# uber/aresdb

Hardware: NVIDIA H100
Metric: rows/s, 1e9-row time-bucketed SUM group-by (cfg3) (higher is better)
Workload: dtype u32/u16/u8 filters; f32 fares summed into f64 (exactly, as integers on the 2^-S grid the zone map allows)

## Files before the change

### aresdb_b200/csrc/batch_plan.cu

```cuda
#include <cooperative_groups.h>
#include <algorithm>
#include <memory>
#include <vector>

#include "agg.cuh"
#include "column.cuh"
#include "dimrow.cuh"
#include "fused_device.cuh"
#include "plan_device.cuh"
#include "radix_sort.cuh"
#include "scan.cuh"
#include "small_sort.cuh"

namespace cg = cooperative_groups;

namespace aresb {

ForeignDesc makeForeignDesc(const ForeignColumnVector &f);
void gatherDims(const uint8_t *in, const DimLayout &Lin, const uint32_t *rows, int g, uint8_t *out,
                const DimLayout &Lout, cudaStream_t s);
int hllRegisterVectors(const uint64_t *hash, const uint32_t *values, uint32_t *index, int R, uint8_t **hllVectorPtr,
                       size_t *hllVectorSizePtr, uint16_t **hllDimRegIDCountPtr, cudaStream_t s);
int reduceByHash(const uint64_t *hash, const uint32_t *index, const uint8_t *measures, int width, AggOp op, int n,
                 uint32_t *outIndex, uint8_t *outValues, cudaStream_t s, uint64_t *outHash = nullptr);
// ... 2021 lines not shown
CGoCallResHandle AggStateFinalizeHLL(void *state, uint8_t **dimValuesPtr, uint8_t **hllVectorPtr, size_t *hllVectorSizePtr,
                                     uint16_t **hllDimRegIDCountPtr, void *cudaStream, int device) {
  return guarded("AggStateFinalizeHLL", device, [&]() -> int64_t {
    return finalizeHLL(asState(state), dimValuesPtr, hllVectorPtr, hllVectorSizePtr, hllDimRegIDCountPtr,
                       (cudaStream_t)cudaStream);
  });
}

CGoCallResHandle AggStateReset(void *state, void *cudaStream, int device) {
  return guarded("AggStateReset", device, [&]() -> int64_t {
    AggState *st = asState(state);
    cudaStream_t s = (cudaStream_t)cudaStream;
    resetClaimedKernel<<<smCount() * 4, 256, 0, s>>>(st->table, st->accNeutral);
    checkLastError("AggStateReset");
    ARES_CUDA(cudaMemsetAsync(st->table.counters, 0, 256, s));
    st->occUpper = 0;
    st->unchecked = 0;
    st->everChecked = false;
    st->resultHost[8] = 0;
    return 0;
  });
}

CGoCallResHandle AresJitDryRun(AggSpec spec, const BatchPlan *plan, char **sourceOut) {
  CGoCallResHandle h = {nullptr, nullptr};
  try {
    AggState st;
    memset(&st.table, 0, sizeof(st.table));
    describeState(&st, spec);
    st.capacity = st.hllDense ? kHllDenseSlots : 0;
    static thread_local DevPlan P;
    compilePlan(&st, *plan, P);
    prepareInputs(P, *plan, nullptr, nullptr);
    layoutStages(P, spec.ExpectedGroups);
    std::string src;
    size_t n = jitCompileOnly(P, &src);
    if (sourceOut) *sourceOut = strdup(src.c_str());
    h.res = reinterpret_cast<void *>(n);
  } catch (const std::exception &e) {
    h.pStrErr = strdup((std::string("AresJitDryRun: ") + e.what()).c_str());
  }
  return h;
}

CGoCallResHandle AresJitDryRunMulti(const AggSpec *specs, int numSpecs, const BatchPlan *plan, char **sourceOut) {
  CGoCallResHandle h = {nullptr, nullptr};
  try {
    if (!specs || !plan || numSpecs < 1 || numSpecs > kJitMaxMeasures) throw EngineError("numSpecs must be 1.." + std::to_string(kJitMaxMeasures));
    std::vector<AggState> st(numSpecs);
    AggState *sts[kJitMaxMeasures];
    for (int k = 0; k < numSpecs; k++) {
      memset(&st[k].table, 0, sizeof(st[k].table));
      describeState(&st[k], specs[k]);
      st[k].capacity = 0;
      sts[k] = &st[k];
    }
    checkSharedStates(sts, numSpecs);
    static thread_local DevPlan P;
    MeasurePlans subs;
    if (numSpecs == 1) {
      compilePlan(sts[0], *plan, P);
      prepareInputs(P, *plan, nullptr, nullptr);
      layoutStages(P, specs[0].ExpectedGroups);
    } else if (!planShared(sts, numSpecs, *plan, P, subs, nullptr, nullptr)) {
      throw EngineError("this plan and zone map run one kernel per state (no shared direct-indexed form)");
    }
// ... 23 lines not shown
```

### aresdb_b200/csrc/jit.cu

```cuda
#include <dlfcn.h>

#include <cassert>
#include <mutex>
#include <sstream>
#include <unordered_map>
#include <vector>
#include <unistd.h>

#include "plan_device.cuh"
#include "jit_embedded.h"

namespace aresb {

typedef struct _nvrtcProgram *nvrtcProgram;
struct Nvrtc {
  int (*CreateProgram)(nvrtcProgram *, const char *, const char *, int, const char *const *, const char *const *);
  int (*CompileProgram)(nvrtcProgram, int, const char *const *);
  int (*GetProgramLogSize)(nvrtcProgram, size_t *);
  int (*GetProgramLog)(nvrtcProgram, char *);
  int (*GetCUBINSize)(nvrtcProgram, size_t *);
  int (*GetCUBIN)(nvrtcProgram, char *);
  int (*DestroyProgram)(nvrtcProgram *);
  bool ok = false;
};
// ... 163 lines not shown
          }
          if (filtered && I.sink == PLAN_SINK_MEASURE && !I.wide && I.nops == 1 && I.fn == Noop && I.akind == 1  && I.aclass == VC_F32 &&
              I.rclass == VC_F32 && I.oclass == VC_F64 && P.cols[I.acol].in.mode != 0 && P.cols[I.acol].rangeKnown) {
            const int e = (int)((P.cols[I.acol].rangeHi >> 23) & 0xFF);
            int S = e == 0 ? 60 : 31 - (e - 127);
            if (S > 60) S = 60;
            if (S < 0) continue;
            P.denseFx = 1;
            P.fxMeasureInst = (int8_t)i;
            P.fxShift = (int8_t)S;
          }
        }
      }
    }
  }
}

static int denseAccOf(uint8_t measWidth, uint8_t aggOp) { return measWidth == 4 && aggOp != OP_MIN_F32 && aggOp != OP_MAX_F32 ? 1 : 2; }
static bool positiveLiteralSum(const DevInst &I, uint8_t aggOp) {
  return I.sink == PLAN_SINK_MEASURE && !I.wide && (aggOp == OP_SUM_I32 || aggOp == OP_SUM_I64) && I.nops == 1 && I.fn == Noop &&
         I.akind == 2  && I.avalid && (I.aclass == VC_I32 || I.aclass == VC_U32) && (int32_t)I.aconst > 0;
}

static void generate(const DevPlan &P, const DevTable &G, Generated &out) {
  const int nmeas = P.nmeas > 1 ? P.nmeas : 1;
  const bool multi = nmeas > 1;
  assert(P.baseCounts == nullptr || P.tileBcBytes != 0 || P.skipCount);
  std::ostringstream os;
  JitParams &jp = out.params;
  memset(&jp, 0, sizeof(jp));
  jp.measureIdentity = P.measureIdentity;
  jp.accNeutral = P.accNeutral;
  jp.G = G;
  jp.ctaAcc = P.ctaAcc;
  jp.numFullTiles = P.numFullTiles;
  jp.numRows = P.numRows;
  jp.join = P.join;
  jp.resume = P.resume;
  jp.startCount = P.startCount;
  int nrle = 0;
  std::vector<int> rleSlot(P.ncols, -1);
  for (int c = 0; c < P.ncols; c++) {
    const DevColumn &col = P.cols[c];
    if (!col.rle) continue;
    assert(nrle < kJitMaxRle && (P.baseCounts == nullptr || P.tileBcBytes != 0));
    rleSlot[c] = nrle;
    jp.rle[nrle].counts = reinterpret_cast<const uint32_t *>(col.in.base);
    jp.rle[nrle].nulls = col.in.base + col.in.nullsOff;
    jp.rle[nrle].values = col.in.base + col.in.valuesOff;
    jp.rle[nrle].tileRun = col.tileRun;
    jp.rle[nrle].length = col.in.length;
    jp.rle[nrle].startBit = col.in.startBit;
    nrle++;
  }

  struct Part { uint32_t off, bytes, stride, isBits, startBit; };
  std::vector<Part> parts;
  size_t tx = 0;
  for (int c = 0; c < P.ncols; c++) {
    const DevColumn &col = P.cols[c];
    if (col.staged) {
      jp.partSrc[parts.size()] = col.in.base + col.in.valuesOff;
      parts.push_back({col.smemValues, col.tileValueBytes, col.width ? P.tileRows * col.width : P.tileRows / 8,
                       col.width ? 0u : 1u, col.in.startBit});
      tx += col.tileValueBytes;
    }
    if (col.hasNulls) {
      jp.partSrc[parts.size()] = col.in.base + col.in.nullsOff;
      parts.push_back({col.smemNulls, col.tileNullBytes, P.tileRows / 8, 1u, col.in.startBit});
      tx += col.tileNullBytes;
    }
  }
  if (P.tileBcBytes != 0) {
    jp.partSrc[parts.size()] = reinterpret_cast<const uint8_t *>(P.baseCounts);
    parts.push_back({P.smemBc, P.tileBcBytes, P.tileRows * 4u, 2u, 0u});
    tx += P.tileBcBytes;
  }
  const bool runLengths = P.tileBcBytes != 0 && !P.skipCount;
  const int kw = P.keyMode == 1  ? 4 : 1;

  struct DenseDim { int inst; bool viaQuot; bool nullCanon; uint32_t lo, cnt, step; bool span32; };
  std::vector<DenseDim> dense;
  std::vector<int> denseOfInst(P.ninsts, -1);
  const bool denseOkPlan = P.denseNd != 0;
  const bool denseOk = denseOkPlan;
  if (denseOk) {
    uint32_t stride = 1;
    for (int k = 0; k < P.denseNd; k++) {
      dense.push_back({P.denseInst[k], P.denseViaQuot[k] != 0, P.denseNullCanon[k] != 0, P.denseLo[k], P.denseCnt[k], P.denseStep[k],
                       P.denseSpan32[k] != 0});
      jp.dBase[k] = P.denseBase[k]; jp.dSpan[k] = P.denseSpan[k];
      jp.dMagic32[k] = P.denseSpan32[k] ? (uint32_t)((1ull << 32) / P.denseStep[k] + 1ull) : 0u;
      denseOfInst[P.denseInst[k]] = k;
      jp.dLo[k] = P.denseLo[k]; jp.dCnt[k] = P.denseCnt[k]; jp.dStep[k] = P.denseStep[k]; jp.dStride[k] = stride;
      stride *= P.denseCnt[k] + 1;
    }
    jp.dTotal = P.denseTotal;
    jp.gAcc = P.denseAcc;
    const uint32_t copyStride = (P.denseTotal + 15) / 16 * 16 + 1;
    uint32_t reps = 1;
    while (!P.denseGlobal && reps < 32 && (uint64_t)copyStride * reps * 2 <= P.smemSlots) reps *= 2;
    jp.dReps = reps;
    jp.dRepStride = reps > 1 ? copyStride : P.denseTotal;
    if (P.hll) { jp.dReps = 1; jp.dRepStride = P.denseTotal; }
    if (P.denseGlobal) {
      jp.dReps = P.denseGlobalReps ? P.denseGlobalReps : 1;
      jp.dRepStride = P.denseTotal;
    }
  }
  int denseAcc = denseAccOf(P.measWidth, P.aggOp);
  int fxMeasure = -1;
  if (denseOk && !P.denseGlobal && P.denseFx) {
    denseAcc = 4;
    fxMeasure = P.fxMeasureInst;
    jp.fxScale = ldexpf(1.0f, P.fxShift);
    jp.fxInv = ldexp(1.0, -P.fxShift);
  }
  bool denseFlags = true, denseCheck = P.neutralSafe;
  for (int i = 0; i < P.ninsts && !multi; i++) {
    if (positiveLiteralSum(P.insts[i], P.aggOp)) {
      denseCheck = false;
      denseFlags = false;
    }
  }
  if (fxMeasure >= 0) denseFlags = false;
  struct MeasForm { int inst, acc; bool flags, check, fx, runLengths; uint8_t aggOp; };
  std::vector<MeasForm> mf;
  if (multi) {
    for (int m = 0; m < nmeas; m++) {
      const DevMeasure &M = P.meas[m];
      const bool lit = positiveLiteralSum(P.insts[M.inst], M.aggOp);
      mf.push_back({M.inst, M.denseFx ? 4 : denseAccOf(M.measWidth, M.aggOp), !lit && !M.denseFx, M.neutralSafe && !lit, M.denseFx != 0,
                    P.tileBcBytes != 0 && !M.skipCount, M.aggOp});
      jp.ms[m].G = M.G;
      jp.ms[m].ctaAcc = M.ctaAcc;
      jp.ms[m].measureIdentity = M.measureIdentity;
      jp.ms[m].accNeutral = M.accNeutral;
      jp.ms[m].fxScale = M.denseFx ? ldexpf(1.0f, M.fxShift) : 0.0f;
      jp.ms[m].fxInv = M.denseFx ? ldexp(1.0, -M.fxShift) : 0.0;
    }
    denseAcc = mf[0].acc; denseFlags = mf[0].flags; denseCheck = mf[0].check;
  } else {
    mf.push_back({-1, denseAcc, denseFlags, denseCheck, false, runLengths, P.aggOp});
  }
  auto measOf = [&](int i) { for (int m = 0; m < nmeas; m++) if (mf[m].inst == i) return m; return 0; };
  auto measName = [](const char *base, int m) { return m ? base + std::to_string(m) : std::string(base); };
  bool anyRunLengths = false;
  for (const MeasForm &f : mf) anyRunLengths = anyRunLengths || f.runLengths;
  for (int k = 0; k < P.denseNd; k++) jp.dStrideB[k] = jp.dStride[k] * (denseOk && denseAcc == 4 && !P.denseGlobal && !multi ? 12u : 1u);
  if (multi) {
    os << "#define JIT_NMEAS " << nmeas << "\n#define JIT_MEAS_REST(v, w)";
    for (int m = 1; m < nmeas; m++) os << " , v[" << m << "], w[" << m << "]";
    os << "\n#define JIT_MEAS_REST1(v)";
    for (int m = 1; m < nmeas; m++) os << " , v[" << m << "]";
    os << "\n";
  }
  os << "#define JIT_DENSE_CHECK " << (denseCheck ? 1 : 0) << "\n";
  os << "#define JIT_DENSE_FLAGS " << (denseFlags ? 1 : 0) << "\n";
  os << "#define JIT_DENSE " << (denseOk ? (P.denseGlobal ? 2 : 1) : 0) << "\n#define JIT_ND " << (denseOk ? dense.size() : 1) << "\n#define JIT_DENSE_ACC "
     << denseAcc << "\n";
  os << "#define JIT_TILE_ROWS " << P.tileRows << "\n#define JIT_STAGE_BYTES " << P.stageBytes
     << "\n#define JIT_STAGE_TX_BYTES " << tx << "\n#define JIT_SMEM_SLOTS " << P.smemSlots << "\n#define JIT_KW " << kw
     << "\n#define JIT_AGG_OP " << (int)P.aggOp << "\n#define JIT_HASH_BITS " << (int)P.hashBits
     << "\n#define JIT_ROW_BYTES " << (int)P.rowBytes << "\n#define JIT_THREADS " << jitThreadsFor(P)
     << "\n#define JIT_STAGES " << P.numStages << "\n#define JIT_HLL " << (int)P.hll << "\n#define JIT_BYPASS " << (int)P.bypassOk
     << "\n#define JIT_DENSE_SLOTS " << P.denseSlots << "\n#define JIT_TABLE_BYTES " << P.tableBytes
     << "\n#define JIT_NUM_PARTS " << parts.size() << "\nnamespace aresb {\n";
  auto table = [&](const char *name, auto get) {
    os << "__device__ constexpr uint32_t " << name << (parts.empty() ? "[1] = {0" : "[JIT_NUM_PARTS] = {");
    for (size_t i = 0; i < parts.size(); i++) os << (i ? ", " : "") << get(parts[i]);
    os << "};\n";
  };
// ... 84 lines not shown
          "__device__ __forceinline__ bool rowEval(const uint8_t *stage, uint32_t q, uint32_t row0, const JitParams &P, uint32_t nvalid,\n"
          "                                        bool (&fast)[4], bool &anySlow, uint32_t (&dslot)[4], uint64_t (&meas)[4],\n"
          "                                        uint32_t (&mraw)[4]" << moreDenseParams << ") {\n"
          "  uint64_t key[4][JIT_KW];   // unused on this path\n"
          "#pragma unroll\n  for (int r = 0; r < 4; r++) mraw[r] = 0;   // float bits of the measure (JIT_DENSE_ACC 4), 0 = not on the integer path\n"
       << moreMrawInit <<
          "  bool din[4] = {true, true, true, true};\n"
          "  anySlow = false;\n"
          "#pragma unroll\n  for (int r = 0; r < 4; r++) { dslot[r] = 0; fast[r] = false; }\n";
  else
    os << (genericForDense ? "// every row with full generality (packed key + measure): the rows the direct-indexed path hands over\nstatic __device__ __noinline__ uint32_t rowEvalGeneric("
                           : "__device__ __forceinline__ uint32_t rowEval(")
       << "const uint8_t *stage, uint32_t q, uint32_t row0, const JitParams &P,\n"
          "                                            uint64_t (&key)[4][JIT_KW], uint64_t (&meas)[4]" << moreGenericParams << ") {\n";
  os << "  bool al[4] = {true, true, true, true};\n"
     << (anyRunLengths ? std::string("  uint32_t runLen[4];   // rows each index position stands for (RLE batch)\n"
                                          "  { const uint32_t *bc = reinterpret_cast<const uint32_t *>(stage + ") + std::to_string(P.smemBc) +
                              ") + 4 * q;\n    const uint4 b = *reinterpret_cast<const uint4 *>(bc); const uint32_t b4 = bc[4];\n"
                              "    runLen[0] = b.y - b.x; runLen[1] = b.z - b.y; runLen[2] = b.w - b.z; runLen[3] = b4 - b.w; }\n"
                            : std::string())
     << "  uint32_t nbAll = 0xFu;   // AND of the null nibbles of the columns that `column CMP literal` filters read\n"
        "#pragma unroll\n  for (int r = 0; r < 4; r++) {\n#pragma unroll\n    for (int k = 0; k < JIT_KW; k++) key[r][k] = 0;\n"
        "    meas[r] = " << (measureAlwaysValid ? "0" : "P.measureIdentity") << ";\n" << moreMeasInit << "  }\n";
  int nconst = 0, nwide = 0, nmagic = 0;
  bool rowsEmitted = false;
  std::vector<bool> colLoaded(P.ncols, false);
  std::vector<int> colConst(P.ncols, -1);
  auto loadColumn = [&](int c) {
    if (colLoaded[c]) return;
    colLoaded[c] = true;
    const DevColumn &col = P.cols[c];
    if (col.in.mode == 0) {
      colConst[c] = nconst;
      jp.consts[nconst++] = (uint32_t)col.in.constLo;
      return;
    }
    if (col.rle) {
      if (!rowsEmitted) {
        rowsEmitted = true;
        if (P.tileBcBytes)
          os << "  uint32_t rowNo[4];\n  { const uint4 b = *reinterpret_cast<const uint4 *>(stage + " << P.smemBc << " + 16 * q);\n"
                "    rowNo[0] = b.x; rowNo[1] = b.y; rowNo[2] = b.z; rowNo[3] = b.w; }\n";
        else
          os << "  uint32_t rowNo[4];\n#pragma unroll\n  for (int r = 0; r < 4; r++) rowNo[r] = P.startCount + row0 + r;\n";
      }
      const bool sgn = col.in.dtype == Int8 || col.in.dtype == Int16;
      os << "  uint32_t c" << c << "[4]; bool cv" << c << "[4]; uint32_t nb" << c << ";\n"
         << "  ldrle<" << (int)col.width << ", " << (sgn ? "true" : "false") << ">(P.rle[" << rleSlot[c] << "], row0 / JIT_TILE_ROWS, rowNo, c" << c
         << ", nb" << c << ");\n#pragma unroll\n  for (int r = 0; r < 4; r++) cv" << c << "[r] = (nb" << c << " & (1u << r)) != 0;\n";
      return;
    }
    assert(col.staged);
    os << "  uint32_t c" << c << "[4]; bool cv" << c << "[4]; uint32_t nb" << c << " = 0xFu;\n";
    if (col.width == 0) {
      os << "  { uint32_t b = ldbits<" << (int)col.in.startBit << ">(stage + " << col.smemValues << ", q);\n"
         << "#pragma unroll\n    for (int r = 0; r < 4; r++) c" << c << "[r] = (b >> r) & 1; }\n";
    } else {
      const bool sgn = col.in.dtype == Int8 || col.in.dtype == Int16;
      os << "  ldq<" << (int)col.width << ", " << (sgn ? "true" : "false") << ">(stage + " << col.smemValues << ", q, c" << c << ");\n";
    }
    if (col.hasNulls)
      os << "  nb" << c << " = ldbits<" << (int)col.in.startBit << ">(stage + " << col.smemNulls << ", q);\n"
         << "#pragma unroll\n  for (int r = 0; r < 4; r++) cv" << c << "[r] = (nb" << c << " & (1u << r)) != 0;\n";
    else
      os << "#pragma unroll\n  for (int r = 0; r < 4; r++) cv" << c << "[r] = true;\n";
  };
  struct Opnd { std::string v, valid; };
  std::vector<int> stack;
  std::vector<bool> ridDone(kMaxForeignTables, false), fcolDone(kMaxForeignCols, false);
  std::vector<std::string> packedTerms;
  auto operand = [&](uint8_t kind, uint8_t colIdx, uint8_t cvalid, uint32_t cbits, Opnd &o) {
    if (kind == 1 ) {
      loadColumn(colIdx);
      if (P.cols[colIdx].in.mode == 0) {
        o.v = "P.consts[" + std::to_string(colConst[colIdx]) + "]";
        o.valid = P.cols[colIdx].in.constValid ? "true" : "false";
      } else {
        o.v = "c" + std::to_string(colIdx) + "[r]";
        o.valid = "cv" + std::to_string(colIdx) + "[r]";
      }
    } else if (kind == 2 ) {
      jp.consts[nconst] = cbits;
      o.v = "P.consts[" + std::to_string(nconst++) + "]";
      o.valid = cvalid ? "true" : "false";
    } else if (kind == 4 ) {
      const int fc = colIdx, t = P.foreignTableOf[fc], jc = P.joinCol[t];
      loadColumn(jc);
      if (!ridDone[t]) {
        ridDone[t] = true;
        os << "  unsigned long long rid" << t << "[4];\n#pragma unroll\n  for (int r = 0; r < 4; r++) rid" << t << "[r] = al[r] && "
           << (P.cols[jc].in.mode == 0 ? std::string(P.cols[jc].in.constValid ? "true" : "false") : "cv" + std::to_string(jc) + "[r]")
           << " ? cuckooLookup(P.join->tables[" << t << "], "
           << (P.cols[jc].in.mode == 0 ? "P.consts[" + std::to_string(colConst[jc]) + "]" : "c" + std::to_string(jc) + "[r]") << ", 0) : 0ull;\n";
      }
      if (!fcolDone[fc]) {
        fcolDone[fc] = true;
        os << "  uint32_t fv" << fc << "[4]; bool fm" << fc << "[4];\n#pragma unroll\n  for (int r = 0; r < 4; r++) {\n"
           << "    Cell f; f.v = 0; f.valid = false;\n    if (al[r]) f = foreignLoad(P.join->cols[" << fc << "], rid" << t << "[r], nullptr);\n"
           << "    fv" << fc << "[r] = (uint32_t)f.v; fm" << fc << "[r] = f.valid;\n  }\n";
      }
      o.v = "fv" + std::to_string(fc) + "[r]";
      o.valid = "fm" + std::to_string(fc) + "[r]";
    } else {
      if (stack.empty()) throw EngineError("plan pops an empty evaluation stack");
      int j = stack.back();
      stack.pop_back();
      o.v = "v" + std::to_string(j) + "[r]";
      o.valid = "m" + std::to_string(j) + "[r]";
    }
  };

  for (int i = 0; i < P.ninsts; i++) {
    const DevInst &I = P.insts[i];
    if (I.wide) {
      const DevColumn &col = P.cols[I.acol];
      const int word = kw == 1 ? 0 : I.rowOff >> 3, sh = (I.rowOff & 7) * 8;
      const int nword = kw == 1 ? 0 : I.nullOff >> 3, nsh = (I.nullOff & 7) * 8;
      if (col.in.mode == 0) {
        auto word64 = [](uint64_t v) { char b[32]; snprintf(b, sizeof(b), "0x%016llxull", (unsigned long long)v); return std::string(b); };
        os << "#pragma unroll\n  for (int r = 0; r < 4; r++) {\n";
        if (I.width == 16)
          os << "    key[r][" << word << "] |= " << word64(col.in.constLo) << ";\n    key[r][" << word + 1 << "] |= " << word64(col.in.constHi) << ";\n";
        else
          os << "    key[r][" << word << "] |= " << word64(col.in.constLo) << (sh ? " << " + std::to_string(sh) : std::string()) << ";\n";
        os << "    key[r][" << nword << "] |= (uint64_t)" << (col.in.constValid ? 1 : 0) << " << " << nsh << ";\n  }\n";
        continue;
      }
      assert((col.in.mode == 1 || col.in.mode == 2) && nwide < kJitMaxWide);
      jp.wideValues[nwide] = col.in.base + col.in.valuesOff;
      jp.wideNulls[nwide] = col.in.mode == 2 ? col.in.base + col.in.nullsOff : nullptr;
      os << "#pragma unroll\n  for (int r = 0; r < 4; r++) {\n    if (row0 + r >= P.numRows) continue;  // tail tile\n"
         << "    const uint64_t *wv = reinterpret_cast<const uint64_t *>(P.wideValues[" << nwide << "]);\n";
      if (I.width == 16) {
        os << "    key[r][" << word << "] |= wv[2 * (size_t)(row0 + r)];\n    key[r][" << word + 1 << "] |= wv[2 * (size_t)(row0 + r) + 1];\n";
      } else {
        os << "    key[r][" << word << "] |= wv[(size_t)(row0 + r)]" << (sh ? " << " + std::to_string(sh) : std::string()) << ";\n";
      }
      if (col.in.mode == 2)
        os << "    key[r][" << nword << "] |= (uint64_t)(bitOf(P.wideNulls[" << nwide << "], row0 + r + " << (int)col.in.startBit
           << ") ? 1 : 0) << " << nsh << ";\n";
      else
        os << "    key[r][" << nword << "] |= (uint64_t)1 << " << nsh << ";\n";
      os << "  }\n";
      nwide++;
      continue;
    }
    Opnd a, b;
    if (I.nops == 2) {
      if (I.bkind == 3) operand(I.bkind, I.bcol, I.bvalid, I.bconst, b);
      operand(I.akind, I.acol, I.avalid, I.aconst, a);
      if (I.bkind != 3) operand(I.bkind, I.bcol, I.bvalid, I.bconst, b);
    } else {
      operand(I.akind, I.acol, I.avalid, I.aconst, a);
    }
    const bool fastDiv = isFastDiv(I) && nmagic < kJitMaxMagic;
    int magicIdx = -1;
    if (fastDiv) {
      magicIdx = nmagic++;
      jp.magic[magicIdx] = magicOk(I) ? (~0ull / I.bconst + 1ull) : 0ull;
    }
    os << "  uint32_t v" << i << "[4]; bool m" << i << "[4];\n";
    const bool fastOnly = fastDiv && magicOk(I);
    const bool spanDiv = denseOk && fastOnly && denseOfInst[i] >= 0 && dense[denseOfInst[i]].viaQuot && dense[denseOfInst[i]].span32 &&
                         I.sink == PLAN_SINK_DIMENSION;
    if (spanDiv) {
      const int k = denseOfInst[i];
      os << "  uint32_t q" << i << "[4]; bool in" << i << "[4];\n#pragma unroll\n  for (int r = 0; r < 4; r++) {\n"
         << "    const uint32_t xr = (uint32_t)cvt(" << a.v << ", " << className(I.aclass) << ", " << className(I.tclass) << ") - P.dBase[" << k << "];\n"
         << "    q" << i << "[r] = __umulhi(xr, P.dMagic32[" << k << "]); in" << i << "[r] = xr < P.dSpan[" << k << "];\n"
         << "    m" << i << "[r] = " << (instValid[i] ? std::string("true") : a.valid) << "; v" << i << "[r] = 0;\n  }\n";
    } else if (fastOnly) {
      const int what = I.fn == Divide ? 0 : I.fn == Mod ? 1 : 2;
      const bool sgn = I.tclass == VC_I32;
      os << "  uint32_t q" << i << "[4];\n  {\n    uint32_t x[4], res[4];\n    const uint32_t d = " << b.v << ";\n"
         << "    const unsigned long long M = P.magic[" << magicIdx << "];\n"
         << "#pragma unroll\n    for (int r = 0; r < 4; r++) x[r] = (uint32_t)cvt(" << a.v << ", " << className(I.aclass) << ", "
         << className(I.tclass) << ");\n"
         << "#pragma unroll\n    for (int r = 0; r < 4; r++) {\n      q" << i << "[r] = fastDivU32(x[r], M);\n"
         << "      res[r] = " << (what == 0 ? "q" + std::to_string(i) + "[r]" : what == 1 ? "x[r] - q" + std::to_string(i) + "[r] * d"
                                                                                         : "q" + std::to_string(i) + "[r] * d") << ";\n    }\n";
      if (sgn)
        os << "    if ((int32_t)(x[0] | x[1] | x[2] | x[3]) < 0) {\n#pragma unroll\n      for (int r = 0; r < 4; r++) res[r] = fastDivOp<" << what
           << ", true>(x[r], d, M);\n    }\n";
// ... 102 lines not shown
    }
  }
  if (denseOk)
    os << "#pragma unroll\n  for (int r = 0; r < 4; r++) {\n    const bool a = al[r] && (uint32_t)r < nvalid;\n"
          "    fast[r] = a && din[r]; anySlow = anySlow || (a && !din[r]);\n  }\n  (void)key;\n  return true;\n}\n";
  else
    os << "  return (al[0] ? 1u : 0u) | (al[1] ? 2u : 0u) | (al[2] ? 4u : 0u) | (al[3] ? 8u : 0u);\n}\n";
  };
  if (denseOkPlan) emitEval(false, 1);
  emitEval(denseOkPlan, 0);
  if (denseOk) {
    os << "__device__ __forceinline__ void densePack(const uint32_t (&dvr)[JIT_ND], uint32_t vb, uint64_t (&key)[JIT_KW]) {\n"
          "#pragma unroll\n  for (int k = 0; k < JIT_KW; k++) key[k] = 0;\n";
    for (size_t k = 0; k < dense.size(); k++) {
      const DevInst &I = P.insts[dense[k].inst];
      const int word = kw == 1 ? 0 : I.rowOff >> 3, sh = (I.rowOff & 7) * 8;
      const int nword = kw == 1 ? 0 : I.nullOff >> 3, nsh = (I.nullOff & 7) * 8;
      os << "  key[" << word << "] |= (uint64_t)dvr[" << k << "] << " << sh << ";\n  key[" << nword << "] |= (uint64_t)((vb >> " << k
         << ") & 1u) << " << nsh << ";\n";
    }
    os << "}\n";
  }
  os << "}  // namespace aresb\n";
  out.source = os.str();
}

struct CompiledKernel {
  cudaLibrary_t lib = nullptr;
  cudaKernel_t kernel = nullptr;
  std::string error;
  bool smemAttr[64] = {false};
};

static std::mutex g_jitMu;
static std::unordered_map<std::string, CompiledKernel *> g_jitCache;
static unsigned long long g_jitCompiles = 0, g_jitLaunches = 0, g_jitDenseLaunches = 0;

static bool readFile(const std::string &path, std::vector<char> &out) {
  FILE *f = fopen(path.c_str(), "rb");
  if (!f) return false;
  fseek(f, 0, SEEK_END);
  long n = ftell(f);
  fseek(f, 0, SEEK_SET);
  out.resize(n > 0 ? (size_t)n : 0);
  const bool ok = n >= 0 && fread(out.data(), 1, out.size(), f) == out.size();
  fclose(f);
  return ok;
// ... 41 lines not shown
    n.DestroyProgram(&prog);
    if (getenv("ARESDB_B200_JIT_DUMP")) fprintf(stderr, "%s\n", src.c_str());
    throw EngineError("NVRTC failed to compile the specialised fused kernel:\n" + log.substr(0, 4000));
  }
  size_t cs = 0;
  n.GetCUBINSize(prog, &cs);
  std::vector<char> cubin(cs);
  n.GetCUBIN(prog, cubin.data());
  n.DestroyProgram(&prog);
  if (!cacheBase.empty()) {
    writeFile(cacheBase + ".cubin", cubin.data(), cubin.size());
    writeFile(cacheBase + ".cu", src.data(), src.size());
  }
  if (const char *dir = getenv("ARESDB_B200_JIT_DUMP_DIR")) {
    static int serial = 0;
    std::string base = std::string(dir) + "/ares_fused_jit_" + std::to_string(serial++);
    if (FILE *f = fopen((base + ".cu").c_str(), "w")) { fwrite(src.data(), 1, src.size(), f); fclose(f); }
    if (FILE *f = fopen((base + ".cubin").c_str(), "wb")) { fwrite(cubin.data(), 1, cubin.size(), f); fclose(f); }
  }
  return cubin;
}

void jitLaunch(const DevPlan &P, const DevTable &G, size_t smemBytes, int grid, cudaStream_t s) {
  Generated gen;
  generate(P, G, gen);
  CompiledKernel *ck = nullptr;
  {
    std::lock_guard<std::mutex> lock(g_jitMu);
    auto it = g_jitCache.find(gen.source);
    if (it == g_jitCache.end()) {
      ck = new CompiledKernel();
      try {
        const std::vector<char> cubin = compileToCubin(gen.source);
        ARES_CUDA(cudaLibraryLoadData(&ck->lib, cubin.data(), nullptr, nullptr, 0, nullptr, nullptr, 0));
        ARES_CUDA(cudaLibraryGetKernel(&ck->kernel, ck->lib, "aresFusedJit"));
        g_jitCompiles++;
      } catch (const std::exception &e) {
        ck->error = e.what();
      }
      it = g_jitCache.emplace(gen.source, ck).first;
    }
    ck = it->second;
    if (!ck->error.empty()) throw EngineError(ck->error);
    int dev = 0;
    cudaGetDevice(&dev);
    if (!ck->smemAttr[dev & 63]) {
      ARES_CUDA(cudaFuncSetAttribute(reinterpret_cast<const void *>(ck->kernel), cudaFuncAttributeMaxDynamicSharedMemorySize,
                                     kSmemBudget));
      ck->smemAttr[dev & 63] = true;
    }
    g_jitLaunches++;
    if (gen.params.dTotal != 0) g_jitDenseLaunches++;
  }
  void *args[] = {&gen.params};
  ARES_CUDA(cudaLaunchKernel(reinterpret_cast<const void *>(ck->kernel), dim3(grid), dim3(jitThreadsFor(P)), args, smemBytes, s));
  noteLaunches(1);
}

size_t jitCompileOnly(const DevPlan &P, std::string *sourceOut) {
  if (!nvrtc().ok) throw EngineError("libnvrtc is not available");
  Generated gen;
  DevTable G;
  memset(&G, 0, sizeof(G));
  generate(P, G, gen);
  if (sourceOut) *sourceOut = gen.source;
  if (getenv("ARESDB_B200_JIT_GENERATE_ONLY")) return gen.source.size();
  return compileToCubin(gen.source).size();
}

}

extern "C" unsigned long long AresJitDenseLaunches() {
  std::lock_guard<std::mutex> lock(aresb::g_jitMu);
  return aresb::g_jitDenseLaunches;
}

extern "C" void AresJitStats(unsigned long long out[2]) {
  std::lock_guard<std::mutex> lock(aresb::g_jitMu);
  out[0] = aresb::g_jitCompiles;
// ... 3 lines not shown
```

### aresdb_b200/csrc/jit_kernel_tail.cuh

```cuda
#ifndef JIT_NMEAS
#define JIT_NMEAS 1
#endif
namespace aresb {

__device__ __forceinline__ void jitIssueTile(const JitParams &P, uint32_t tile, uint8_t *stage, uint64_t *bar) {
  mbarExpectTx(bar, JIT_STAGE_TX_BYTES);
#pragma unroll
  for (int p = 0; p < JIT_NUM_PARTS; p++)
    tmaLoad1D(stage + kPartSmemOff[p], P.partSrc[p] + (size_t)tile * kPartTileStride[p], kPartBytes[p], bar);
}

__device__ __forceinline__ unsigned long long jitKeyOfRow(const uint64_t (&key)[JIT_KW]) {
  if (JIT_KW == 1) return key[0];
  uint64_t w[4] = {key[0], key[JIT_KW > 1 ? 1 : 0], key[JIT_KW > 2 ? 2 : 0], key[JIT_KW > 3 ? 3 : 0]};
  return JIT_HASH_BITS == 64 ? murmur3_128_lo(w, JIT_ROW_BYTES, 0) : (unsigned long long)murmur3_32(w, JIT_ROW_BYTES, 0);
}
__device__ __forceinline__ unsigned long long jitKeyOf(const uint64_t (&key)[4][JIT_KW], const uint64_t (&meas)[4], int r) {
  unsigned long long k = jitKeyOfRow(key[r]);
  if (JIT_HLL == 1) k = (k & 0xFFFFFFFFFFFF0000ull) | (meas[r] & 0x3FFFu);
  return k;
}

#if JIT_DENSE
#if JIT_NMEAS == 1
// ... 573 lines not shown
  for (uint32_t i = threadIdx.x; i < denseSlots; i += JIT_THREADS) {
    unsigned long long accS = P.accNeutral;
    if (JIT_DENSE_ACC == 4) {
      const uint32_t *c = reinterpret_cast<const uint32_t *>(tKeys) + 3u * i;
      const unsigned long long v = (unsigned long long)c[0] + ((unsigned long long)c[1] << 11) + ((unsigned long long)c[2] << 22);
      if (v != 0) accS = (unsigned long long)__double_as_longlong(__ull2double_rn(v) * P.fxInv);
    } else {
      accS = denseSharedAcc()[i];
    }
    const unsigned long long accG = JIT_DENSE_ACC != 1 ? __ldcg(&tAcc[i]) : P.accNeutral;
    if (JIT_DENSE_FLAGS ? !touched[i] : (accS == P.accNeutral && accG == P.accNeutral)) continue;
    uint32_t rem = i % P.dRepStride, dvr[JIT_ND], vb = 0;
#pragma unroll
    for (int k = JIT_ND - 1; k >= 0; k--) {
      const uint32_t ix = rem / P.dStride[k];
      rem -= ix * P.dStride[k];
      const bool valid = ix != P.dCnt[k];
      dvr[k] = valid ? (P.dLo[k] + ix) * P.dStep[k] : 0u;
      vb |= (valid ? 1u : 0u) << k;
    }
    uint64_t key[JIT_KW];
    densePack(dvr, vb, key);
    const unsigned long long k = jitKeyOfRow(key);
    if (JIT_DENSE_ACC != 1) globalUpdate(P.G, (AggOp)JIT_AGG_OP, k, JIT_KW == 1 ? nullptr : key, accG, true);
    globalUpdate(P.G, (AggOp)JIT_AGG_OP, k, JIT_KW == 1 ? nullptr : key, accS, true);
  }
  return;
#endif
  for (uint32_t i = threadIdx.x; i < JIT_SMEM_SLOTS; i += JIT_THREADS) {
    unsigned long long k = tKeys[i];
    if (k != kEmptyKey) globalUpdate(P.G, (AggOp)JIT_AGG_OP, k, nullptr, __ldcg(&tAcc[i]), true);
  }
  if (blockIdx.x == 0 && threadIdx.x == 0) *P.G.occPublish = *reinterpret_cast<volatile uint32_t *>(&P.G.counters[0]);
}

}
```

### aresdb_b200/csrc/plan_device.cuh

```cuda
#pragma once
#include "column.cuh"
#include "fused_device.cuh"
#include "jit_params.cuh"
#include "join.cuh"

namespace aresb {

constexpr int kSmemBudget = 232448;
constexpr int kJitThreads = 1024;
constexpr int kMaxGridCtas = 160;
static_assert(kMaxPlanInsts == ARES_MAX_PLAN_INSTS && kMaxForeignTables == ARES_MAX_FOREIGN_TABLES &&
              kMaxForeignCols == ARES_MAX_FOREIGN_COLUMNS, "jit_params.cuh restates the plan bounds of batch_plan.h");

enum KeyMode : uint8_t { KEY_PACKED = 0, KEY_HASHED = 1 };
enum OperandKind : uint8_t { OPK_NONE = 0, OPK_COLUMN = 1, OPK_CONST = 2, OPK_STACK = 3, OPK_FOREIGN = 4 };

struct DevColumn {
  InputDesc in;
  uint32_t smemValues;
  uint32_t smemNulls;
  uint32_t tileValueBytes;
  uint32_t tileNullBytes;
  uint8_t width;
  uint8_t staged;
// ... 60 lines not shown
  uint8_t denseGlobalReps;
  uint8_t neutralSafe;
  uint8_t denseFx;
  int8_t fxMeasureInst;
  int8_t fxShift;
  uint8_t numForeignTables, numForeignCols;
  uint8_t joinCol[kMaxForeignTables];
  uint8_t foreignTableOf[kMaxForeignCols];
  uint8_t foreignClass[kMaxForeignCols];
  uint8_t pad2[1];
  const DevJoin *join;
  uint32_t resume;
  uint8_t nmeas;
  DevMeasure meas[kJitMaxMeasures];
};

constexpr uint32_t kDenseMaxSlots = 8192;
constexpr uint32_t kFxMaxRowsPerCta = 1u << 21;
constexpr uint32_t kGlobalDenseMaxSlots = 1u << 21;

void jitAnalyzeDense(DevPlan &P, bool bypass);
size_t jitCompileOnly(const DevPlan &P, std::string *sourceOut);
void jitLaunch(const DevPlan &P, const DevTable &G, size_t smemBytes, int grid, cudaStream_t s);

}
```

Before: 240.5 billion.

## Key JIT kernel cache by plan shape instead of rendered source text

Splits kernel generation into parameter filling and source rendering. The launch path now builds a compact binary shape key and looks up the compiled kernel with it, so the full CUDA source no longer has to be rendered and hashed on every launch. Source is rendered only on a cache miss. It also skips a global update of the second dense accumulator when that accumulator still holds the neutral value. It adds a dry-run entry point that checks the key and parameters, and it risks a wrong cache hit if the key misses something the generated source depends on.

```diff
diff --git a/aresdb_b200/csrc/batch_plan.cu b/aresdb_b200/csrc/batch_plan.cu
--- a/aresdb_b200/csrc/batch_plan.cu
+++ b/aresdb_b200/csrc/batch_plan.cu
@@ -2067,17 +2067,22 @@
   });
 }
 
+static const DevPlan &dryRunPlan(const AggSpec &spec, const BatchPlan &plan) {
+  AggState st;
+  memset(&st.table, 0, sizeof(st.table));
+  describeState(&st, spec);
+  st.capacity = st.hllDense ? kHllDenseSlots : 0;
+  static thread_local DevPlan P;
+  compilePlan(&st, plan, P);
+  prepareInputs(P, plan, nullptr, nullptr);
+  layoutStages(P, spec.ExpectedGroups);
+  return P;
+}
+
 CGoCallResHandle AresJitDryRun(AggSpec spec, const BatchPlan *plan, char **sourceOut) {
   CGoCallResHandle h = {nullptr, nullptr};
   try {
-    AggState st;
-    memset(&st.table, 0, sizeof(st.table));
-    describeState(&st, spec);
-    st.capacity = st.hllDense ? kHllDenseSlots : 0;
-    static thread_local DevPlan P;
-    compilePlan(&st, *plan, P);
-    prepareInputs(P, *plan, nullptr, nullptr);
-    layoutStages(P, spec.ExpectedGroups);
+    const DevPlan &P = dryRunPlan(spec, *plan);
     std::string src;
     size_t n = jitCompileOnly(P, &src);
     if (sourceOut) *sourceOut = strdup(src.c_str());
@@ -2087,6 +2092,25 @@
   }
   return h;
 }
+
+CGoCallResHandle AresJitDryRunShape(AggSpec spec, const BatchPlan *plan, char **keyOut, char **sourceOut, void *launchParams,
+                                    void *generatedParams) {
+  CGoCallResHandle h = {nullptr, nullptr};
+  try {
+    if (!plan || !keyOut || !sourceOut || !launchParams || !generatedParams) throw EngineError("arguments must not be null");
+    std::string key, src;
+    jitShapeOnly(dryRunPlan(spec, *plan), key, src, *static_cast<JitParams *>(launchParams), *static_cast<JitParams *>(generatedParams));
+    *keyOut = static_cast<char *>(malloc(key.size() ? key.size() : 1));
+    memcpy(*keyOut, key.data(), key.size());
+    *sourceOut = strdup(src.c_str());
+    h.res = reinterpret_cast<void *>(key.size());
+  } catch (const std::exception &e) {
+    h.pStrErr = strdup((std::string("AresJitDryRunShape: ") + e.what()).c_str());
+  }
+  return h;
+}
+
+size_t AresJitParamsSize() { return sizeof(JitParams); }
 
 CGoCallResHandle AresJitDryRunMulti(const AggSpec *specs, int numSpecs, const BatchPlan *plan, char **sourceOut) {
   CGoCallResHandle h = {nullptr, nullptr};
diff --git a/aresdb_b200/csrc/jit.cu b/aresdb_b200/csrc/jit.cu
--- a/aresdb_b200/csrc/jit.cu
+++ b/aresdb_b200/csrc/jit.cu
@@ -209,12 +209,34 @@
          I.akind == 2  && I.avalid && (I.aclass == VC_I32 || I.aclass == VC_U32) && (int32_t)I.aconst > 0;
 }
 
-static void generate(const DevPlan &P, const DevTable &G, Generated &out) {
-  const int nmeas = P.nmeas > 1 ? P.nmeas : 1;
-  const bool multi = nmeas > 1;
-  assert(P.baseCounts == nullptr || P.tileBcBytes != 0 || P.skipCount);
-  std::ostringstream os;
-  JitParams &jp = out.params;
+struct Part { uint32_t off, bytes, stride, isBits, startBit; const uint8_t *src; };
+static std::vector<Part> stagedParts(const DevPlan &P) {
+  std::vector<Part> parts;
+  for (int c = 0; c < P.ncols; c++) {
+    const DevColumn &col = P.cols[c];
+    if (col.staged)
+      parts.push_back({col.smemValues, col.tileValueBytes, col.width ? P.tileRows * col.width : P.tileRows / 8, col.width ? 0u : 1u,
+                       col.in.startBit, col.in.base + col.in.valuesOff});
+    if (col.hasNulls) parts.push_back({col.smemNulls, col.tileNullBytes, P.tileRows / 8, 1u, col.in.startBit, col.in.base + col.in.nullsOff});
+  }
+  if (P.tileBcBytes != 0)
+    parts.push_back({P.smemBc, P.tileBcBytes, P.tileRows * 4u, 2u, 0u, reinterpret_cast<const uint8_t *>(P.baseCounts)});
+  return parts;
+}
+
+static int denseAccOfPlan(const DevPlan &P) {
+  return P.denseNd != 0 && !P.denseGlobal && P.denseFx ? 4 : denseAccOf(P.measWidth, P.aggOp);
+}
+
+struct ParamSlots {
+  int rle[kMaxPlanCols];
+  int colConst[kMaxPlanCols];
+  int aconst[kMaxPlanInsts], bconst[kMaxPlanInsts];
+  int magic[kMaxPlanInsts];
+  int wide[kMaxPlanInsts];
+};
+
+static void fillParams(const DevPlan &P, const DevTable &G, JitParams &jp, ParamSlots &sl) {
   memset(&jp, 0, sizeof(jp));
   jp.measureIdentity = P.measureIdentity;
   jp.accNeutral = P.accNeutral;
@@ -226,12 +248,12 @@
   jp.resume = P.resume;
   jp.startCount = P.startCount;
   int nrle = 0;
-  std::vector<int> rleSlot(P.ncols, -1);
+  for (int c = 0; c < kMaxPlanCols; c++) sl.rle[c] = sl.colConst[c] = -1;
   for (int c = 0; c < P.ncols; c++) {
     const DevColumn &col = P.cols[c];
     if (!col.rle) continue;
     assert(nrle < kJitMaxRle && (P.baseCounts == nullptr || P.tileBcBytes != 0));
-    rleSlot[c] = nrle;
+    sl.rle[c] = nrle;
     jp.rle[nrle].counts = reinterpret_cast<const uint32_t *>(col.in.base);
     jp.rle[nrle].nulls = col.in.base + col.in.nullsOff;
     jp.rle[nrle].values = col.in.base + col.in.valuesOff;
@@ -240,46 +262,18 @@
     jp.rle[nrle].startBit = col.in.startBit;
     nrle++;
   }
-
-  struct Part { uint32_t off, bytes, stride, isBits, startBit; };
-  std::vector<Part> parts;
-  size_t tx = 0;
-  for (int c = 0; c < P.ncols; c++) {
-    const DevColumn &col = P.cols[c];
-    if (col.staged) {
-      jp.partSrc[parts.size()] = col.in.base + col.in.valuesOff;
-      parts.push_back({col.smemValues, col.tileValueBytes, col.width ? P.tileRows * col.width : P.tileRows / 8,
-                       col.width ? 0u : 1u, col.in.startBit});
-      tx += col.tileValueBytes;
-    }
-    if (col.hasNulls) {
-      jp.partSrc[parts.size()] = col.in.base + col.in.nullsOff;
-      parts.push_back({col.smemNulls, col.tileNullBytes, P.tileRows / 8, 1u, col.in.startBit});
-      tx += col.tileNullBytes;
-    }
-  }
-  if (P.tileBcBytes != 0) {
-    jp.partSrc[parts.size()] = reinterpret_cast<const uint8_t *>(P.baseCounts);
-    parts.push_back({P.smemBc, P.tileBcBytes, P.tileRows * 4u, 2u, 0u});
-    tx += P.tileBcBytes;
-  }
-  const bool runLengths = P.tileBcBytes != 0 && !P.skipCount;
-  const int kw = P.keyMode == 1  ? 4 : 1;
-
-  struct DenseDim { int inst; bool viaQuot; bool nullCanon; uint32_t lo, cnt, step; bool span32; };
-  std::vector<DenseDim> dense;
-  std::vector<int> denseOfInst(P.ninsts, -1);
-  const bool denseOkPlan = P.denseNd != 0;
-  const bool denseOk = denseOkPlan;
-  if (denseOk) {
+  const std::vector<Part> parts = stagedParts(P);
+  for (size_t i = 0; i < parts.size(); i++) jp.partSrc[i] = parts[i].src;
+
+  const bool multi = P.nmeas > 1;
+  const int denseAcc = denseAccOfPlan(P);
+  if (P.denseNd != 0) {
     uint32_t stride = 1;
     for (int k = 0; k < P.denseNd; k++) {
-      dense.push_back({P.denseInst[k], P.denseViaQuot[k] != 0, P.denseNullCanon[k] != 0, P.denseLo[k], P.denseCnt[k], P.denseStep[k],
-                       P.denseSpan32[k] != 0});
       jp.dBase[k] = P.denseBase[k]; jp.dSpan[k] = P.denseSpan[k];
       jp.dMagic32[k] = P.denseSpan32[k] ? (uint32_t)((1ull << 32) / P.denseStep[k] + 1ull) : 0u;
-      denseOfInst[P.denseInst[k]] = k;
       jp.dLo[k] = P.denseLo[k]; jp.dCnt[k] = P.denseCnt[k]; jp.dStep[k] = P.denseStep[k]; jp.dStride[k] = stride;
+      jp.dStrideB[k] = stride * (denseAcc == 4 && !multi ? 12u : 1u);
       stride *= P.denseCnt[k] + 1;
     }
     jp.dTotal = P.denseTotal;
@@ -295,14 +289,127 @@
       jp.dRepStride = P.denseTotal;
     }
   }
-  int denseAcc = denseAccOf(P.measWidth, P.aggOp);
-  int fxMeasure = -1;
-  if (denseOk && !P.denseGlobal && P.denseFx) {
-    denseAcc = 4;
-    fxMeasure = P.fxMeasureInst;
+  if (denseAcc == 4) {
     jp.fxScale = ldexpf(1.0f, P.fxShift);
     jp.fxInv = ldexp(1.0, -P.fxShift);
   }
+  for (int m = 0; multi && m < P.nmeas; m++) {
+    const DevMeasure &M = P.meas[m];
+    jp.ms[m].G = M.G;
+    jp.ms[m].ctaAcc = M.ctaAcc;
+    jp.ms[m].measureIdentity = M.measureIdentity;
+    jp.ms[m].accNeutral = M.accNeutral;
+    jp.ms[m].fxScale = M.denseFx ? ldexpf(1.0f, M.fxShift) : 0.0f;
+    jp.ms[m].fxInv = M.denseFx ? ldexp(1.0, -M.fxShift) : 0.0;
+  }
+
+  int nconst = 0, nwide = 0, nmagic = 0;
+  bool colLoaded[kMaxPlanCols] = {false};
+  auto loadColumn = [&](int c) {
+    if (colLoaded[c]) return;
+    colLoaded[c] = true;
+    if (P.cols[c].in.mode == 0) {
+      sl.colConst[c] = nconst;
+      jp.consts[nconst++] = (uint32_t)P.cols[c].in.constLo;
+    }
+  };
+  auto operand = [&](uint8_t kind, uint8_t colIdx, uint32_t cbits, int &slot) {
+    slot = -1;
+    if (kind == 1 ) loadColumn(colIdx);
+    else if (kind == 4 ) loadColumn(P.joinCol[P.foreignTableOf[colIdx]]);
+    else if (kind == 2 ) { slot = nconst; jp.consts[nconst++] = cbits; }
+  };
+  for (int i = 0; i < P.ninsts; i++) {
+    const DevInst &I = P.insts[i];
+    sl.aconst[i] = sl.bconst[i] = sl.magic[i] = sl.wide[i] = -1;
+    if (I.wide) {
+      const DevColumn &col = P.cols[I.acol];
+      if (col.in.mode == 0) continue;
+      assert((col.in.mode == 1 || col.in.mode == 2) && nwide < kJitMaxWide);
+      sl.wide[i] = nwide;
+      jp.wideValues[nwide] = col.in.base + col.in.valuesOff;
+      jp.wideNulls[nwide] = col.in.mode == 2 ? col.in.base + col.in.nullsOff : nullptr;
+      nwide++;
+      continue;
+    }
+    if (I.nops == 2) {
+      if (I.bkind == 3) operand(I.bkind, I.bcol, I.bconst, sl.bconst[i]);
+      operand(I.akind, I.acol, I.aconst, sl.aconst[i]);
+      if (I.bkind != 3) operand(I.bkind, I.bcol, I.bconst, sl.bconst[i]);
+    } else {
+      operand(I.akind, I.acol, I.aconst, sl.aconst[i]);
+    }
+    if (isFastDiv(I) && nmagic < kJitMaxMagic) {
+      sl.magic[i] = nmagic;
+      jp.magic[nmagic++] = magicOk(I) ? (~0ull / I.bconst + 1ull) : 0ull;
+    }
+  }
+}
+
+static void shapeKey(const DevPlan &P, std::string &key) {
+  key.clear();
+  auto put = [&](const void *p, size_t n) { key.append(static_cast<const char *>(p), n); };
+  auto put32 = [&](uint32_t v) { put(&v, 4); };
+  const uint32_t head[] = {(uint32_t)P.ncols, (uint32_t)P.ninsts, (uint32_t)P.lastFilter, P.tileRows, P.stageBytes, P.smemSlots,
+                           P.numStages, P.denseSlots, P.smemBc, P.tileBcBytes, P.tableBytes,
+                           (uint32_t)P.keyMode | (uint32_t)P.rowBytes << 8 | (uint32_t)P.hashBits << 16 | (uint32_t)P.aggOp << 24,
+                           (uint32_t)P.measWidth | (uint32_t)P.skipCount << 8 | (uint32_t)P.hll << 16 | (uint32_t)P.bypassOk << 24,
+                           (uint32_t)P.denseNd | (uint32_t)P.denseGlobal << 8 | (uint32_t)P.denseFx << 16 | (uint32_t)(uint8_t)P.fxMeasureInst << 24,
+                           (uint32_t)P.neutralSafe | (uint32_t)(P.nmeas > 1 ? P.nmeas : 1) << 8};
+  put(head, sizeof(head));
+  for (int k = 0; k < P.denseNd; k++)
+    put32((uint32_t)P.denseInst[k] | (uint32_t)P.denseViaQuot[k] << 8 | (uint32_t)P.denseNullCanon[k] << 16 | (uint32_t)P.denseSpan32[k] << 24);
+  for (int c = 0; c < P.ncols; c++) {
+    const DevColumn &col = P.cols[c];
+    const uint32_t w[] = {col.smemValues, col.smemNulls, col.tileValueBytes, col.tileNullBytes,
+                          (uint32_t)col.width | (uint32_t)col.staged << 8 | (uint32_t)col.hasNulls << 16 | (uint32_t)col.rle << 24,
+                          (uint32_t)col.in.mode | (uint32_t)col.in.constValid << 8 | (uint32_t)col.in.dtype << 16, col.in.startBit};
+    put(w, sizeof(w));
+  }
+  for (int i = 0; i < P.ninsts; i++) {
+    DevInst I = P.insts[i];
+    const uint8_t decided = (uint8_t)((isFastDiv(I) && magicOk(I) ? 1 : 0) | (positiveLiteralSum(I, P.aggOp) ? 2 : 0));
+    if (I.wide && P.cols[I.acol].in.mode == 0) { put(&P.cols[I.acol].in.constLo, 8); put(&P.cols[I.acol].in.constHi, 8); }
+    if (I.akind == 4 || I.bkind == 4) {
+      const uint8_t fc = I.akind == 4 ? I.acol : I.bcol, t = P.foreignTableOf[fc];
+      put(&t, 1); put(&P.joinCol[t], 1);
+      if (I.akind == 4 && I.bkind == 4) { put(&P.foreignTableOf[I.bcol], 1); put(&P.joinCol[P.foreignTableOf[I.bcol]], 1); }
+    }
+    I.aconst = I.bconst = 0;
+    I.pad = decided;
+    put(&I, sizeof(I));
+  }
+  for (int m = 0; P.nmeas > 1 && m < P.nmeas; m++) {
+    const DevMeasure &M = P.meas[m];
+    const uint8_t w[] = {(uint8_t)M.inst, M.aggOp, M.measWidth, M.skipCount, M.neutralSafe, M.denseFx,
+                         (uint8_t)positiveLiteralSum(P.insts[M.inst], M.aggOp)};
+    put(w, sizeof(w));
+  }
+}
+
+static std::string renderSource(const DevPlan &P, const ParamSlots &sl) {
+  const int nmeas = P.nmeas > 1 ? P.nmeas : 1;
+  const bool multi = nmeas > 1;
+  assert(P.baseCounts == nullptr || P.tileBcBytes != 0 || P.skipCount);
+  std::ostringstream os;
+
+  const std::vector<Part> parts = stagedParts(P);
+  size_t tx = 0;
+  for (const Part &p : parts) tx += p.bytes;
+  const bool runLengths = P.tileBcBytes != 0 && !P.skipCount;
+  const int kw = P.keyMode == 1  ? 4 : 1;
+
+  struct DenseDim { int inst; bool viaQuot; bool nullCanon; bool span32; };
+  std::vector<DenseDim> dense;
+  std::vector<int> denseOfInst(P.ninsts, -1);
+  const bool denseOkPlan = P.denseNd != 0;
+  const bool denseOk = denseOkPlan;
+  for (int k = 0; k < P.denseNd; k++) {
+    dense.push_back({P.denseInst[k], P.denseViaQuot[k] != 0, P.denseNullCanon[k] != 0, P.denseSpan32[k] != 0});
+    denseOfInst[P.denseInst[k]] = k;
+  }
+  int denseAcc = denseAccOfPlan(P);
+  const int fxMeasure = denseAcc == 4 ? P.fxMeasureInst : -1;
   bool denseFlags = true, denseCheck = P.neutralSafe;
   for (int i = 0; i < P.ninsts && !multi; i++) {
     if (positiveLiteralSum(P.insts[i], P.aggOp)) {
@@ -319,12 +426,6 @@
       const bool lit = positiveLiteralSum(P.insts[M.inst], M.aggOp);
       mf.push_back({M.inst, M.denseFx ? 4 : denseAccOf(M.measWidth, M.aggOp), !lit && !M.denseFx, M.neutralSafe && !lit, M.denseFx != 0,
                     P.tileBcBytes != 0 && !M.skipCount, M.aggOp});
-      jp.ms[m].G = M.G;
-      jp.ms[m].ctaAcc = M.ctaAcc;
-      jp.ms[m].measureIdentity = M.measureIdentity;
-      jp.ms[m].accNeutral = M.accNeutral;
-      jp.ms[m].fxScale = M.denseFx ? ldexpf(1.0f, M.fxShift) : 0.0f;
-      jp.ms[m].fxInv = M.denseFx ? ldexp(1.0, -M.fxShift) : 0.0;
     }
     denseAcc = mf[0].acc; denseFlags = mf[0].flags; denseCheck = mf[0].check;
   } else {
@@ -334,7 +435,6 @@
   auto measName = [](const char *base, int m) { return m ? base + std::to_string(m) : std::string(base); };
   bool anyRunLengths = false;
   for (const MeasForm &f : mf) anyRunLengths = anyRunLengths || f.runLengths;
-  for (int k = 0; k < P.denseNd; k++) jp.dStrideB[k] = jp.dStride[k] * (denseOk && denseAcc == 4 && !P.denseGlobal && !multi ? 12u : 1u);
   if (multi) {
     os << "#define JIT_NMEAS " << nmeas << "\n#define JIT_MEAS_REST(v, w)";
     for (int m = 1; m < nmeas; m++) os << " , v[" << m << "], w[" << m << "]";
@@ -465,19 +565,13 @@
      << "  uint32_t nbAll = 0xFu;   // AND of the null nibbles of the columns that `column CMP literal` filters read\n"
         "#pragma unroll\n  for (int r = 0; r < 4; r++) {\n#pragma unroll\n    for (int k = 0; k < JIT_KW; k++) key[r][k] = 0;\n"
         "    meas[r] = " << (measureAlwaysValid ? "0" : "P.measureIdentity") << ";\n" << moreMeasInit << "  }\n";
-  int nconst = 0, nwide = 0, nmagic = 0;
   bool rowsEmitted = false;
   std::vector<bool> colLoaded(P.ncols, false);
-  std::vector<int> colConst(P.ncols, -1);
   auto loadColumn = [&](int c) {
     if (colLoaded[c]) return;
     colLoaded[c] = true;
     const DevColumn &col = P.cols[c];
-    if (col.in.mode == 0) {
-      colConst[c] = nconst;
-      jp.consts[nconst++] = (uint32_t)col.in.constLo;
-      return;
-    }
+    if (col.in.mode == 0) return;
     if (col.rle) {
       if (!rowsEmitted) {
         rowsEmitted = true;
@@ -489,7 +583,7 @@
       }
       const bool sgn = col.in.dtype == Int8 || col.in.dtype == Int16;
       os << "  uint32_t c" << c << "[4]; bool cv" << c << "[4]; uint32_t nb" << c << ";\n"
-         << "  ldrle<" << (int)col.width << ", " << (sgn ? "true" : "false") << ">(P.rle[" << rleSlot[c] << "], row0 / JIT_TILE_ROWS, rowNo, c" << c
+         << "  ldrle<" << (int)col.width << ", " << (sgn ? "true" : "false") << ">(P.rle[" << sl.rle[c] << "], row0 / JIT_TILE_ROWS, rowNo, c" << c
          << ", nb" << c << ");\n#pragma unroll\n  for (int r = 0; r < 4; r++) cv" << c << "[r] = (nb" << c << " & (1u << r)) != 0;\n";
       return;
     }
@@ -512,19 +606,18 @@
   std::vector<int> stack;
   std::vector<bool> ridDone(kMaxForeignTables, false), fcolDone(kMaxForeignCols, false);
   std::vector<std::string> packedTerms;
-  auto operand = [&](uint8_t kind, uint8_t colIdx, uint8_t cvalid, uint32_t cbits, Opnd &o) {
+  auto operand = [&](uint8_t kind, uint8_t colIdx, uint8_t cvalid, int constSlot, Opnd &o) {
     if (kind == 1 ) {
       loadColumn(colIdx);
       if (P.cols[colIdx].in.mode == 0) {
-        o.v = "P.consts[" + std::to_string(colConst[colIdx]) + "]";
+        o.v = "P.consts[" + std::to_string(sl.colConst[colIdx]) + "]";
         o.valid = P.cols[colIdx].in.constValid ? "true" : "false";
       } else {
         o.v = "c" + std::to_string(colIdx) + "[r]";
         o.valid = "cv" + std::to_string(colIdx) + "[r]";
       }
     } else if (kind == 2 ) {
-      jp.consts[nconst] = cbits;
-      o.v = "P.consts[" + std::to_string(nconst++) + "]";
+      o.v = "P.consts[" + std::to_string(constSlot) + "]";
       o.valid = cvalid ? "true" : "false";
     } else if (kind == 4 ) {
       const int fc = colIdx, t = P.foreignTableOf[fc], jc = P.joinCol[t];
@@ -534,7 +627,7 @@
         os << "  unsigned long long rid" << t << "[4];\n#pragma unroll\n  for (int r = 0; r < 4; r++) rid" << t << "[r] = al[r] && "
            << (P.cols[jc].in.mode == 0 ? std::string(P.cols[jc].in.constValid ? "true" : "false") : "cv" + std::to_string(jc) + "[r]")
            << " ? cuckooLookup(P.join->tables[" << t << "], "
-           << (P.cols[jc].in.mode == 0 ? "P.consts[" + std::to_string(colConst[jc]) + "]" : "c" + std::to_string(jc) + "[r]") << ", 0) : 0ull;\n";
+           << (P.cols[jc].in.mode == 0 ? "P.consts[" + std::to_string(sl.colConst[jc]) + "]" : "c" + std::to_string(jc) + "[r]") << ", 0) : 0ull;\n";
       }
       if (!fcolDone[fc]) {
         fcolDone[fc] = true;
@@ -569,9 +662,7 @@
         os << "    key[r][" << nword << "] |= (uint64_t)" << (col.in.constValid ? 1 : 0) << " << " << nsh << ";\n  }\n";
         continue;
       }
-      assert((col.in.mode == 1 || col.in.mode == 2) && nwide < kJitMaxWide);
-      jp.wideValues[nwide] = col.in.base + col.in.valuesOff;
-      jp.wideNulls[nwide] = col.in.mode == 2 ? col.in.base + col.in.nullsOff : nullptr;
+      const int nwide = sl.wide[i];
       os << "#pragma unroll\n  for (int r = 0; r < 4; r++) {\n    if (row0 + r >= P.numRows) continue;  // tail tile\n"
          << "    const uint64_t *wv = reinterpret_cast<const uint64_t *>(P.wideValues[" << nwide << "]);\n";
       if (I.width == 16) {
@@ -585,23 +676,18 @@
       else
         os << "    key[r][" << nword << "] |= (uint64_t)1 << " << nsh << ";\n";
       os << "  }\n";
-      nwide++;
       continue;
     }
     Opnd a, b;
     if (I.nops == 2) {
-      if (I.bkind == 3) operand(I.bkind, I.bcol, I.bvalid, I.bconst, b);
-      operand(I.akind, I.acol, I.avalid, I.aconst, a);
-      if (I.bkind != 3) operand(I.bkind, I.bcol, I.bvalid, I.bconst, b);
+      if (I.bkind == 3) operand(I.bkind, I.bcol, I.bvalid, sl.bconst[i], b);
+      operand(I.akind, I.acol, I.avalid, sl.aconst[i], a);
+      if (I.bkind != 3) operand(I.bkind, I.bcol, I.bvalid, sl.bconst[i], b);
     } else {
-      operand(I.akind, I.acol, I.avalid, I.aconst, a);
-    }
-    const bool fastDiv = isFastDiv(I) && nmagic < kJitMaxMagic;
-    int magicIdx = -1;
-    if (fastDiv) {
-      magicIdx = nmagic++;
-      jp.magic[magicIdx] = magicOk(I) ? (~0ull / I.bconst + 1ull) : 0ull;
-    }
+      operand(I.akind, I.acol, I.avalid, sl.aconst[i], a);
+    }
+    const int magicIdx = sl.magic[i];
+    const bool fastDiv = magicIdx >= 0;
     os << "  uint32_t v" << i << "[4]; bool m" << i << "[4];\n";
     const bool fastOnly = fastDiv && magicOk(I);
     const bool spanDiv = denseOk && fastOnly && denseOfInst[i] >= 0 && dense[denseOfInst[i]].viaQuot && dense[denseOfInst[i]].span32 &&
@@ -750,7 +836,13 @@
     os << "}\n";
   }
   os << "}  // namespace aresb\n";
-  out.source = os.str();
+  return os.str();
+}
+
+static void generate(const DevPlan &P, const DevTable &G, Generated &out) {
+  ParamSlots sl;
+  fillParams(P, G, out.params, sl);
+  out.source = renderSource(P, sl);
 }
 
 struct CompiledKernel {
@@ -838,23 +930,26 @@
 }
 
 void jitLaunch(const DevPlan &P, const DevTable &G, size_t smemBytes, int grid, cudaStream_t s) {
-  Generated gen;
-  generate(P, G, gen);
+  static thread_local std::string key;
+  shapeKey(P, key);
+  JitParams params;
+  ParamSlots sl;
+  fillParams(P, G, params, sl);
   CompiledKernel *ck = nullptr;
   {
     std::lock_guard<std::mutex> lock(g_jitMu);
-    auto it = g_jitCache.find(gen.source);
+    auto it = g_jitCache.find(key);
     if (it == g_jitCache.end()) {
       ck = new CompiledKernel();
       try {
-        const std::vector<char> cubin = compileToCubin(gen.source);
+        const std::vector<char> cubin = compileToCubin(renderSource(P, sl));
         ARES_CUDA(cudaLibraryLoadData(&ck->lib, cubin.data(), nullptr, nullptr, 0, nullptr, nullptr, 0));
         ARES_CUDA(cudaLibraryGetKernel(&ck->kernel, ck->lib, "aresFusedJit"));
         g_jitCompiles++;
       } catch (const std::exception &e) {
         ck->error = e.what();
       }
-      it = g_jitCache.emplace(gen.source, ck).first;
+      it = g_jitCache.emplace(key, ck).first;
     }
     ck = it->second;
     if (!ck->error.empty()) throw EngineError(ck->error);
@@ -866,11 +961,23 @@
       ck->smemAttr[dev & 63] = true;
     }
     g_jitLaunches++;
-    if (gen.params.dTotal != 0) g_jitDenseLaunches++;
-  }
-  void *args[] = {&gen.params};
+    if (params.dTotal != 0) g_jitDenseLaunches++;
+  }
+  void *args[] = {&params};
   ARES_CUDA(cudaLaunchKernel(reinterpret_cast<const void *>(ck->kernel), dim3(grid), dim3(jitThreadsFor(P)), args, smemBytes, s));
   noteLaunches(1);
+}
+
+void jitShapeOnly(const DevPlan &P, std::string &key, std::string &source, JitParams &launchParams, JitParams &generatedParams) {
+  DevTable G;
+  memset(&G, 0, sizeof(G));
+  shapeKey(P, key);
+  ParamSlots sl;
+  fillParams(P, G, launchParams, sl);
+  Generated gen;
+  generate(P, G, gen);
+  source = gen.source;
+  generatedParams = gen.params;
 }
 
 size_t jitCompileOnly(const DevPlan &P, std::string *sourceOut) {
diff --git a/aresdb_b200/csrc/jit_kernel_tail.cuh b/aresdb_b200/csrc/jit_kernel_tail.cuh
--- a/aresdb_b200/csrc/jit_kernel_tail.cuh
+++ b/aresdb_b200/csrc/jit_kernel_tail.cuh
@@ -619,7 +619,7 @@
     uint64_t key[JIT_KW];
     densePack(dvr, vb, key);
     const unsigned long long k = jitKeyOfRow(key);
-    if (JIT_DENSE_ACC != 1) globalUpdate(P.G, (AggOp)JIT_AGG_OP, k, JIT_KW == 1 ? nullptr : key, accG, true);
+    if (JIT_DENSE_ACC != 1 && accG != P.accNeutral) globalUpdate(P.G, (AggOp)JIT_AGG_OP, k, JIT_KW == 1 ? nullptr : key, accG, true);
     globalUpdate(P.G, (AggOp)JIT_AGG_OP, k, JIT_KW == 1 ? nullptr : key, accS, true);
   }
   return;
diff --git a/aresdb_b200/csrc/plan_device.cuh b/aresdb_b200/csrc/plan_device.cuh
--- a/aresdb_b200/csrc/plan_device.cuh
+++ b/aresdb_b200/csrc/plan_device.cuh
@@ -106,5 +106,6 @@
 void jitAnalyzeDense(DevPlan &P, bool bypass);
 size_t jitCompileOnly(const DevPlan &P, std::string *sourceOut);
 void jitLaunch(const DevPlan &P, const DevTable &G, size_t smemBytes, int grid, cudaStream_t s);
+void jitShapeOnly(const DevPlan &P, std::string &key, std::string &source, JitParams &launchParams, JitParams &generatedParams);
 
 }
```

Result: faster. 247.2 billion (median of 6 runs) (+2.8%).
